# NeymarL/ChineseChess-AlphaZero

Measured on AMD Instinct MI355X. Metric: mcts_node_expansions_per_sec, higher is better.
Workload: dtype f16+2xbf6corr-split/f32acc+f64/i32 tree

## Files before the change

### chinesechess-alphazero_amd/cchess_alphazero/_native.py

```python
import ctypes as C
import os

import numpy as np

_HERE = os.path.dirname(os.path.abspath(__file__))
LIB_PATH = os.environ.get("CZ_LIB") or os.path.join(os.path.dirname(_HERE), "csrc", "libczero.so")

NSQ, NLABELS, MAXMOVES, NOMOVE = 90, 2086, 128, 0xFFFF
F32, F16, BF16, U8, F16C8, F16C6, F16C86 = 0, 1, 2, 3, 4, 5, 6

_lib = None


class NativeError(RuntimeError):
    pass


def lib():
    global _lib
    if _lib is None:
        import torch
        if not os.path.exists(LIB_PATH):
            raise NativeError(
                f"{LIB_PATH} not found: build the HIP engine first "
# ... 34 lines not shown
        L.cz_input_conv.argtypes = [vp, i32, i32, vp, vp, vp, vp, i32, i32, i32, i32, i32, vp]
        L.cz_input_conv.restype = i32
        L.cz_input_conv_packed_elems.argtypes = [i32, i32, i32]
        L.cz_input_conv_packed_elems.restype = C.c_size_t
        L.cz_input_conv_pack_weights.argtypes = [vp, i32, i32, i32, i32, vp]
        L.cz_input_conv_pack_weights.restype = i32
        L.cz_resblock_heads.argtypes = [vp, vp, vp, vp, vp, vp, vp, vp, vp, vp, i32, i32, i32, i32, i32, vp]
        L.cz_resblock_heads.restype = i32
        L.cz_resblock.argtypes = [vp, vp, vp, vp, vp, vp, vp, vp, vp, i32, i32, i32, i32, vp]
        L.cz_input_conv_q.argtypes = [vp, i32, i32, vp, vp, vp, vp, i32, i32, i32, i32, i32, vp, vp, vp]
        L.cz_resblock_q.argtypes = [vp, vp, vp, vp, vp, vp, vp, vp, vp, i32, i32, i32, i32, vp, vp]
        L.cz_resblock_heads_q.argtypes = [vp, vp, vp, vp, vp, vp, vp, vp, vp, vp, i32, i32, i32, i32, i32, vp, vp]
        for _n in ("cz_input_conv_q", "cz_resblock_q", "cz_resblock_heads_q"):
            getattr(L, _n).restype = i32
        L.cz_resblock.restype = i32
        L.cz_split_bias_act.argtypes = [vp, vp, vp, vp, C.c_size_t, i32, i32, i32, i32, vp]
        L.cz_split_bias_act.restype = i32
    if hasattr(L, "cz_conv3x3_c8"):
        L.cz_conv3x3_c8_packed_bytes.argtypes = [i32]
        L.cz_conv3x3_c8_packed_bytes.restype = C.c_size_t
        L.cz_conv3x3_c8_pack_weights.argtypes = [vp, i32, vp]
        L.cz_conv3x3_c8_pack_weights.restype = i32
        L.cz_conv3x3_c6_pack_weights.argtypes = [vp, i32, i32, i32, vp]
        L.cz_conv3x3_c6_pack_weights.restype = i32
        L.cz_conv3x3_c8.argtypes = [vp, vp, vp, vp, vp, vp, vp, vp, vp, i32, i32, i32, vp]
        L.cz_conv3x3_c8.restype = i32
    if hasattr(L, "cz_input_resblock"):
        L.cz_input_resblock.argtypes = [vp, i32, vp, vp, vp, vp, vp, vp, vp, vp, i32, i32, i32, vp, vp, vp]
        L.cz_input_resblock.restype = i32
    if hasattr(L, "cz_tower"):
        L.cz_input_resblock_m.restype = i32
        L.cz_input_resblock_m.argtypes = [vp, vp, i32] + [vp] * 8 + [i32] * 3 + [vp] * 3
        L.cz_tower.restype = i32
        L.cz_tower.argtypes = [vp, vp, i32, vp, vp, vp, vp, vp, vp, i32, vp, vp, vp, vp, vp, vp, i32, i32, i32, vp, vp]
        L.cz_resblock_chain.restype = i32
        L.cz_resblock_chain.argtypes = [vp, vp, i32, vp, vp, vp, vp, vp, vp, vp, i32, i32, i32, vp, vp]
        L.cz_tower_plain.restype = i32
        L.cz_tower_plain.argtypes = [vp, i32, vp, vp, vp, vp, vp, i32, i32, i32, vp, vp]
        L.cz_tower_pairs.restype = i32
        L.cz_tower_pairs.argtypes = [vp, vp, i32, vp, vp, vp, vp, vp, vp, vp, vp, vp, vp, i32, i32, i32, i32, vp, vp]
    if hasattr(L, "cz_heads_tail"):
        L.cz_heads_tail.argtypes = [vp, i32, vp, vp, i32, vp, i32, vp, vp, i32, vp, C.c_float, vp, vp, vp, i32, i32, i32, vp, vp]
        L.cz_heads_tail.restype = i32
        L.cz_fc_packed_elems.argtypes = [i32, i32]
        L.cz_fc_packed_elems.restype = C.c_size_t
        L.cz_fc_pack_weights.argtypes = [vp, i32, i32, i32, vp]
        L.cz_fc_pack_weights.restype = i32
    for name in ("cz_label_tables", "cz_movegen", "cz_done", "cz_step", "cz_encode", "cz_check_or_catch",
                 "cz_be_catched", "cz_has_attack", "cz_rules_fused"):
        getattr(L, name).restype = i32
    if hasattr(L, "cz_replay_games"):
        L.cz_replay_games.argtypes = [vp, vp, vp, i32, i32, vp, vp, vp, vp]
        L.cz_replay_games.restype = i32
    if hasattr(L, "cz_gather_planes"):
        L.cz_gather_planes.argtypes = [vp, vp, i32, vp, i32, i32, vp, vp]
        L.cz_gather_planes.restype = i32
    if hasattr(L, "cz_policy_value_loss"):
        L.cz_policy_value_loss.argtypes = [vp, i32, vp, vp, i32, i32, vp, vp, vp, i32, vp, vp, i32, C.c_float, C.c_float,
                                           vp, vp, vp, vp, vp]
        L.cz_policy_value_loss.restype = i32
    if hasattr(L, "cz_search_create"):
        from . import _native_search
        _native_search.declare(L)


def check(rc, what=""):
# ... 280 lines not shown
    return out_f32 if out_f32 is not None else out


def head_convs(x, w, bias, n_policy, policy_feat, value_feat):
    require_gpu()
    n, c = x.shape[0], x.shape[-1]
    check(lib().cz_head_convs(_ptr(x), _dt_code(x.dtype), _ptr(w), _ptr(bias), _ptr(policy_feat), _ptr(value_feat),
                              n, c, n_policy, w.shape[0] - n_policy, _stream()), "cz_head_convs")
    return policy_feat, value_feat


def input_table(w_oihw):
    import torch
    w = w_oihw.detach().to(torch.float32)
    return w.permute(1, 2, 3, 0).reshape(w.shape[1], 25, w.shape[0]).contiguous()


def input_resblock(planes, table, in_bias, w1, b1, w2, b2, out, rows=None, count=None, masks=None):
    require_gpu()
    import torch
    if planes.dtype != torch.uint8:
        raise NativeError("cz_input_resblock reads uint8 planes")
    n = planes.shape[0]
    if masks is not None:
        assert masks.dtype == torch.int32 and masks.is_cuda and masks.is_contiguous() and tuple(masks.shape) == (n, 96)
    L = lib()
    check(L.cz_input_resblock_m(_ptr(planes), _ptr(masks), planes.shape[1], _ptr(table), _ptr(in_bias), _ptr(w1), _ptr(b1),
                                _ptr(w2), _ptr(b2), _ptr(out[0]), _ptr(out[1]), n, out[0].shape[-1], _pair_code(out),
                                _ptr(rows) if rows is not None else None, _ptr(count) if count is not None else None,
                                _stream()), "cz_input_resblock")
    return out


def pack_fc_weights(w, dtype=None):
    import torch
    dtype = dtype or torch.float16
    w = w.detach().to("cpu", torch.float32).contiguous()
    n = lib().cz_fc_packed_elems(w.shape[0], w.shape[1])
    if n == 0:
        raise NativeError(f"cz_fc_pack_weights: unsupported shape {tuple(w.shape)}")
    out = torch.empty((n,), dtype=dtype)
    check(lib().cz_fc_pack_weights(_ptr(w), w.shape[0], w.shape[1], _dt_code(dtype), _ptr(out)), "cz_fc_pack_weights")
    return out


def heads_tail(policy_feat, value_feat, wp, bias_p, w1, bias1, w2, b2, policy, value, stats, count=None, normalize=True):
    require_gpu()
    n = policy_feat.shape[0]
    check(lib().cz_heads_tail(_ptr(policy_feat), policy_feat.shape[1], _ptr(wp), _ptr(bias_p), policy.shape[1],
                              _ptr(value_feat), value_feat.shape[1], _ptr(w1), _ptr(bias1), bias1.shape[0], _ptr(w2),
                              float(b2), _ptr(policy), _ptr(value), _ptr(stats), n, _dt_code(wp.dtype), int(bool(normalize)),
                              _ptr(count) if count is not None else None, _stream()), "cz_heads_tail")
    return policy, value


def pack_input_conv_weights(w_oihw, dtype, parts):
    import torch
    w = w_oihw.detach().to("cpu", torch.float32).contiguous()
    c, ip = w.shape[0], w.shape[1]
    assert tuple(w.shape[2:]) == (5, 5)
    n = lib().cz_input_conv_packed_elems(c, ip, parts)
    if n == 0:
        raise NativeError(f"cz_input_conv: unsupported channels={c} in_planes={ip} parts={parts}")
    out = torch.empty((n,), dtype=dtype)
    check(lib().cz_input_conv_pack_weights(_ptr(w), c, ip, _dt_code(dtype), parts, _ptr(out)),
          "cz_input_conv_pack_weights")
# ... 150 lines not shown
```

### chinesechess-alphazero_amd/cchess_alphazero/agent/model.py

```python
import hashlib
import json
import os
from logging import getLogger

import torch
import torch.nn as nn
import torch.nn.functional as F

logger = getLogger(__name__)

N_LABELS = 2086
BN_EPS = 1e-3


class ResidualBlock(nn.Module):
    def __init__(self, filters, ksize):
        super().__init__()
        self.conv1 = nn.Conv2d(filters, filters, ksize, padding=ksize // 2, bias=False)
        self.bn1 = nn.BatchNorm2d(filters, eps=BN_EPS, momentum=0.01)
        self.conv2 = nn.Conv2d(filters, filters, ksize, padding=ksize // 2, bias=False)
        self.bn2 = nn.BatchNorm2d(filters, eps=BN_EPS, momentum=0.01)

    def forward(self, x):
        y = F.relu(self.bn1(self.conv1(x)))
# ... 126 lines not shown
        self.c6_blocks = 0
        if arith == "c6" or arith.startswith("c6>"):
            n6 = int(arith[3:]) if arith.startswith("c6>") else nblk
            assert 1 <= n6 <= nblk, arith
            self.c6 = (trunk == "mfma" and dtype == torch.float32 and net.cfg["cnn_filter_num"] in (128, 192) and nblk >= 2)
            if self.c6 and act_exps is None:
                if not from_env:
                    raise ValueError("arith='c6' needs the activation images' exponents: build the network through "
                                     "guarded_inference_net (it measures them on the calibration positions)")
                logger.warning("CZ_TOWER_ARITH=%s without calibrated exponents: using c8 (guarded_inference_net measures them)", arith)
                self.c6 = False
            self.c6_blocks = n6 if self.c6 else 0
            arith = "c8"
        self.act_exps = ([int(v) for v in act_exps[0]], [int(v) for v in act_exps[1]]) if self.c6 else None
        if arith.startswith("c8"):
            c8_blocks = int(arith[3:]) if arith.startswith("c8>") else nblk
            assert 0 <= c8_blocks <= nblk, arith
            if not (trunk == "mfma" and dtype == torch.float32 and net.cfg["cnn_filter_num"] in (128, 192)):
                c8_blocks = 0
            arith = "c8" if c8_blocks else "f16x3"
        assert arith in ("bf16x3", "f16x3", "c8"), arith
        if arith == "f16x3" and not (trunk == "mfma" and dtype == torch.float32):
            arith = "bf16x3"
        self.arith = arith
        self.c8_blocks = c8_blocks
        self.fused_epilogue = True
        self.fused_blocks = True
        self.fused_heads = True
        self.fused_input = os.environ.get("CZ_FUSED_INPUT", "1") != "0"
        self.fused_tail = os.environ.get("CZ_FUSED_TAIL", "1") != "0"
        self.block_events = None
        self.last_plan = None
        self.chain_blocks = os.environ.get("CZ_TOWER_CHAIN", "1") != "0"
        self.chain_heads = os.environ.get("CZ_TOWER_HEADS", "1") != "0"
        self.input_depth = net.cfg["input_depth"]
        self.filters = net.cfg["cnn_filter_num"]
        with torch.no_grad():
            self.input_conv = _fold(net.input_conv, net.input_bn)
            self.res = nn.ModuleList()
            for blk in net.res:
                self.res.append(nn.ModuleList([_fold(blk.conv1, blk.bn1), _fold(blk.conv2, blk.bn2)]))
            self.policy_conv = _fold(net.policy_conv, net.policy_bn)
            self.value_conv = _fold(net.value_conv, net.value_bn)
            self.policy_out = nn.Linear(net.policy_out.in_features, net.policy_out.out_features)
            self.value_dense = nn.Linear(net.value_dense.in_features, net.value_dense.out_features)
            self.value_out = nn.Linear(net.value_out.in_features, 1)
            self.policy_out.load_state_dict(net.policy_out.state_dict())
            self.value_dense.load_state_dict(net.value_dense.state_dict())
            self.value_out.load_state_dict(net.value_out.state_dict())
            self.act_shift = None
            if act_shift is not None and (act_shift[0] != 0 or any(act_shift[1])):
                sx, smid = int(act_shift[0]), [int(v) for v in act_shift[1]]
                assert len(smid) == len(self.res)
                self.act_shift = (sx, smid)
                self.input_conv.weight.mul_(2.0 ** sx)
                self.input_conv.bias.mul_(2.0 ** sx)
                for (c1, c2), sm in zip(self.res, smid):
                    c1.weight.mul_(2.0 ** (sm - sx))
                    c1.bias.mul_(2.0 ** sm)
                    c2.weight.mul_(2.0 ** (sx - sm))
                    c2.bias.mul_(2.0 ** sx)
                self.policy_conv.weight.mul_(2.0 ** -sx)
                self.value_conv.weight.mul_(2.0 ** -sx)
            packed = self._pack_trunk() if trunk == "mfma" else None
        self.to(dtype)
        self.to(memory_format=torch.channels_last)
# ... 172 lines not shown
                cur, tmp, nxt = (self._as_f16_pair(t) for t in (cur, tmp, nxt))
                _native.split_bias_act(last, None, cur, relu=False)
            conv = _native.conv3x3_c8 if i < n8 else _native.conv3x3
            conv(cur, w1, getattr(self, f"tb{i}a"), out=tmp)
            if i + 1 < nblk and i + 1 != n8:
                conv(tmp, w2, getattr(self, f"tb{i}b"), skip=cur, out=nxt)
                cur, nxt = nxt, cur
            elif self.parts == 2:
                conv(tmp, w2, getattr(self, f"tb{i}b"), skip=cur, out_f32=last)
            else:
                conv(tmp, w2, getattr(self, f"tb{i}b"), skip=cur, out=(last,))
        if heads is not None and fused and self.parts == 2 and c == 128:
            return None
        return last

    def block_kinds(self):
        nblk = len(self.res)
        if self.c6:
            return ["c6"] * self.c6_blocks + ["c8"] * (nblk - self.c6_blocks)
        if self.arith == "c8":
            return ["c8"] * self.c8_blocks + ["pair"] * (nblk - self.c8_blocks)
        return ["pair"] * nblk

    def _block_params(self, i):
        od = self.operand_dtype
        return (getattr(self, f"tw{i}a").view(od), getattr(self, f"tb{i}a"), getattr(self, f"tw{i}b").view(od), getattr(self, f"tb{i}b"))

    def _tower_chained(self, planes, cur, nxt, last, heads, rows, count, masks):
        from cchess_alphazero import _native
        kinds = self.block_kinds()
        nblk = len(kinds)
        heads_ok = heads is not None and self.parts == 2 and self.filters == 128
        chain_heads = self.chain_heads and not (kinds[-1] == "pair" and self.operand_dtype == torch.bfloat16)
        key = ("plan", heads_ok, chain_heads, self.tb0a.data_ptr())
        if key not in self._bufs:
            plan = []
            for step in tower_plan(kinds, heads_exit=heads_ok, chain_heads=chain_heads):
                if step[0] in ("tower", "pairs"):
                    blk = step[1]
                    fmt = [_native.IMG_C6 if kinds[blk[0]] == "c6" else _native.IMG_C8] * len(blk)
                    bl = _native.BlockList([self._block_params(i) for i in blk], *((fmt, fmt) if step[0] == "tower" else ()))
                    plan.append(step + (bl,))
                else:
                    plan.append(step)
            self._bufs[key] = plan
        self.last_plan = [st[:3] if st[0] != "first" else st for st in self._bufs[key]]
        img_tag = {"c6": torch.int8, "c8": torch.uint8}

        def view(t, kind):
            if kind == "pair":
                return (t[0], t[1].view(t[0].dtype)) if t[1].dtype in (torch.uint8, torch.int8) else t
            return (t[0], t[1].view(img_tag[kind]))
        fmt_code = {"c6": _native.IMG_C6, "c8": _native.IMG_C8, "pair": _native.IMG_PAIR}
        hd = (self.head_w32, self.head_b32, heads[0], heads[1], heads[2]) if heads_ok else None
        done_heads = False
        for step in self._bufs[key]:
            ev = None
            if self.block_events is not None:
                ev = (torch.cuda.Event(enable_timing=True), torch.cuda.Event(enable_timing=True))
                ev[0].record()
            if step[0] == "first":
                w1, b1, w2, b2 = self._block_params(0)
                _native.input_resblock(planes.contiguous(), self.in_table32, self.in_bias32, w1, b1, w2, b2,
                                       out=view(nxt, kinds[0]), rows=rows, count=count, masks=masks)
                cur, nxt = nxt, cur
                nb = 1
            elif step[0] == "tower":
                _, blk, ex, bl = step
                nb = len(blk)
                if ex == "heads":
                    _native.tower(view(cur, kinds[blk[0]]), bl, _native.EXIT_HEADS, heads=hd, count=count)
                    done_heads = True
                else:
                    _native.tower(view(cur, kinds[blk[0]]), bl, fmt_code[ex], out=view(nxt, ex), count=count)
                    cur, nxt = nxt, cur
            elif step[0] == "pairs":
                _, blk, with_heads, bl = step
                nb = len(blk)
                if with_heads:
                    _native.tower_pairs(view(cur, "pair"), bl, heads=hd, count=count)
                    done_heads = True
                else:
                    _native.tower_pairs(view(cur, "pair"), bl, out=view(nxt, "pair"), count=count)
                    cur, nxt = nxt, cur
            else:
                i = step[1]
                nb = 1
                w1, b1, w2, b2 = self._block_params(i)
                x = view(cur, kinds[i])
                if heads_ok:
                    _native.resblock_heads(x, w1, b1, w2, b2, self.head_w32, self.head_b32, heads[0], heads[1], heads[2],
                                           count=count)
                    done_heads = True
                else:
                    _native.resblock(x, w1, b1, w2, b2, out_f32=last, count=count)
            if ev is not None:
                ev[1].record()
                self.block_events.append(ev + (nb,) if nb > 1 else ev)
        return None if done_heads else last

    def _tower_192(self, cur, nxt, last, count):
        from cchess_alphazero import _native
        kinds = self.block_kinds()
        nblk = len(kinds)
        legacy = os.environ.get("CZ_IP_PAIR", "1")[:1] == "0"
        key = ("plan192", legacy, self.tb0a.data_ptr())
        if key not in self._bufs:
# ... 518 lines not shown
```

### chinesechess-alphazero_amd/csrc/xq_conv.hip

```cpp
#include <hip/hip_runtime.h>
#include <stdint.h>
#include <string.h>
#include <stdlib.h>
#include <stdio.h>
#include <math.h>
#include "../../include/czero.h"
#include "xq_c8_kloop.h"
#include "xq_nn_common.h"

extern "C" void czi_set_error(const char* msg);
extern "C" int czi_pairs4_launch(const void* x_hi, const void* x_lo, int n_blocks, const void* const* w1, const float* const* b1,
                                 const void* const* w2, const float* const* b2, void* y_hi, void* y_lo, const float* head_w,
                                 const float* head_b, float* pol, float* val, int n_pol, int n_boards, int channels, int dtype,
                                 int n_cu, const int32_t* n_dev, void* stream, float* y_f32);

namespace {

struct QueueCtx {
    const int32_t* rows = nullptr;
    const int32_t* n_dev = nullptr;
};
thread_local QueueCtx g_q;

template <int C, int P, int PARTS> struct Geom {
// ... 3285 lines not shown
                               (const unsigned char*)x_img, ch, (_Float16*)y_hi, (unsigned char*)y_img, y_f32, n_boards, n_dev, 0, HeadArgs{});
        else
            hipLaunchKernelGGL((k_resblock_ip4_c8<192, 1, 1>), dim3(blocks), dim3(256), 0, st, (const _Float16*)x_hi,
                               (const unsigned char*)x_img, ch, (_Float16*)y_hi, (unsigned char*)y_img, y_f32, n_boards, n_dev, 0, HeadArgs{});
    } else {
        const unsigned blocks = (unsigned)(n_boards < n_cu ? n_boards : n_cu);
        if (dtype == CZ_F16C8)
            hipLaunchKernelGGL((k_resblock_ip_c8<192, 0, 0>), dim3(blocks), dim3(192 / 32 * 64 + ip::COPY_THREADS), 0, st, (const _Float16*)x_hi,
                               (const unsigned char*)x_img, ch, (_Float16*)y_hi, (unsigned char*)y_img, y_f32, n_boards, n_dev);
        else
            hipLaunchKernelGGL((k_resblock_ip_c8<192, 1, 1>), dim3(blocks), dim3(192 / 32 * 64 + ip::COPY_THREADS), 0, st, (const _Float16*)x_hi,
                               (const unsigned char*)x_img, ch, (_Float16*)y_hi, (unsigned char*)y_img, y_f32, n_boards, n_dev);
    }
    if (hipGetLastError() != hipSuccess) {
        czi_set_error("cz_resblock_chain: launch failed");
        return CZ_ERR_HIP;
    }
    return CZ_OK;
}

extern "C" int czi_tower4_launch(const void* x_hi, const void* x_img, int n_blocks, const void* const* w1, const float* const* b1,
                                 const void* const* w2, const float* const* b2, int c6, int exit_mode, void* y_hi, void* y_img,
                                 const float* head_w, const float* head_b, float* pol, float* val, int n_pol, int n_boards,
                                 int n_cu, const int32_t* n_dev, void* stream)
{
    if (n_blocks > ip::MAX_BLOCKS) return CZ_ERR_ARG;
    const HeadArgs hd{head_w, head_b, pol, val, n_pol};
    hipStream_t st = (hipStream_t)stream;
    ip::Chain ch{};
    ch.n = n_blocks;
    for (int b = 0; b < n_blocks; ++b) { ch.w1[b] = w1[b]; ch.w2[b] = w2[b]; ch.b1[b] = b1[b]; ch.b2[b] = b2[b]; }
    const int n_pairs = (n_boards + 1) / 2;
    const unsigned blocks = (unsigned)(n_pairs < n_cu ? n_pairs : n_cu);
    if (c6)
        hipLaunchKernelGGL((k_resblock_ip4_c8<128, 1, 1>), dim3(blocks), dim3(256), 0, st, (const _Float16*)x_hi, (const unsigned char*)x_img,
                           ch, (_Float16*)y_hi, (unsigned char*)y_img, (float*)nullptr, n_boards, n_dev, exit_mode, hd);
    else
        hipLaunchKernelGGL((k_resblock_ip4_c8<128, 0, 0>), dim3(blocks), dim3(256), 0, st, (const _Float16*)x_hi, (const unsigned char*)x_img,
                           ch, (_Float16*)y_hi, (unsigned char*)y_img, (float*)nullptr, n_boards, n_dev, exit_mode, hd);
    return hipGetLastError() == hipSuccess ? CZ_OK : CZ_ERR_HIP;
}

extern "C" int cz_tower_plain(const void* x, int n_blocks, const void* const* w1_packed, const float* const* bias1,
                              const void* const* w2_packed, const float* const* bias2, void* y, int n_boards, int channels,
                              int dtype, const int32_t* n_dev, void* stream)
{
    if (n_boards < 0 || !x || !y || !w1_packed || !w2_packed || !bias1 || !bias2 || n_blocks < 1 || n_blocks > pl::MAX_BLOCKS ||
        channels != 256 || (dtype != CZ_F16 && dtype != CZ_BF16)) {
        czi_set_error("cz_tower_plain: bad argument (256 filters, plain f16 / bf16 operands, 1 .. 24 blocks)");
        return CZ_ERR_ARG;
    }
    pl::Chain ch{};
    ch.n = n_blocks;
    for (int b = 0; b < n_blocks; ++b) {
        if (!w1_packed[b] || !w2_packed[b] || !bias1[b] || !bias2[b]) {
            czi_set_error("cz_tower_plain: null block parameter");
            return CZ_ERR_ARG;
        }
        ch.w1[b] = w1_packed[b]; ch.w2[b] = w2_packed[b]; ch.b1[b] = bias1[b]; ch.b2[b] = bias2[b];
    }
    if (n_boards == 0) return CZ_OK;
    const int n_cu = device_cu_count();
    if (n_cu < 0) {
        czi_set_error("cz_tower_plain: cannot query the device");
        return CZ_ERR_HIP;
    }
    hipStream_t st = (hipStream_t)stream;
// ... 45 lines not shown
    if (n_cu < 0) {
        czi_set_error("cz_input_resblock: cannot query the device");
        return CZ_ERR_HIP;
    }
    hipStream_t st = (hipStream_t)stream;
    const unsigned blocks = (unsigned)(n_boards < n_cu ? n_boards : n_cu);
    const FirstArgs fa{(const unsigned char*)planes_u8, in_table, in_bias, rows, masks, in_planes, g_first_w1_rounds};
    if (dtype == CZ_F16C6) {
        if (launch_resblock_c8<true, false, true>(nullptr, nullptr, w1_packed, bias1, w2_packed, bias2, y_hi, y_lo, nullptr,
                                                  n_boards, n_cu, st, HeadArgs{}, n_dev, fa) != CZ_OK) {
            czi_set_error("cz_input_resblock: launch failed");
            return CZ_ERR_HIP;
        }
        return CZ_OK;
    }
    if (dtype == CZ_F16C8) {
        if (launch_resblock_c8<true, false>(nullptr, nullptr, w1_packed, bias1, w2_packed, bias2, y_hi, y_lo, nullptr, n_boards,
                                            n_cu, st, HeadArgs{}, n_dev, fa) != CZ_OK) {
            czi_set_error("cz_input_resblock: launch failed");
            return CZ_ERR_HIP;
        }
        return CZ_OK;
    }
    if (dtype == CZ_BF16)
        hipLaunchKernelGGL((k_resblock_pipe<__bf16, true>), dim3(blocks), dim3(512), 0, st, (const __bf16*)nullptr,
                           (const __bf16*)nullptr, (const __bf16*)w1_packed, bias1, (const __bf16*)w2_packed, bias2,
                           (__bf16*)y_hi, (__bf16*)y_lo, n_boards, n_dev, fa);
    else
        hipLaunchKernelGGL((k_resblock_pipe<_Float16, true>), dim3(blocks), dim3(512), 0, st, (const _Float16*)nullptr,
                           (const _Float16*)nullptr, (const _Float16*)w1_packed, bias1, (const _Float16*)w2_packed, bias2,
                           (_Float16*)y_hi, (_Float16*)y_lo, n_boards, n_dev, fa);
    if (hipGetLastError() != hipSuccess) {
        czi_set_error("cz_input_resblock: launch failed");
        return CZ_ERR_HIP;
    }
    return CZ_OK;
}

extern "C" int cz_resblock_pipelined(int enable)
{
    const int old = g_resblock_pipelined;
    if (enable >= 0) g_resblock_pipelined = enable ? 1 : 0;
    return old;
}

extern "C" int cz_input_conv_q(const void* planes, int planes_dtype, int in_planes, const void* w_packed,
                               const float* bias, void* y_hi, void* y_lo, int n_boards, int channels, int dtype,
                               int parts, int relu, const int32_t* rows, const int32_t* n_dev, void* stream)
{
    g_q = QueueCtx{rows, n_dev};
    const int rc = cz_input_conv(planes, planes_dtype, in_planes, w_packed, bias, y_hi, y_lo, n_boards, channels, dtype,
                                 parts, relu, stream);
    g_q = QueueCtx{};
    return rc;
}

extern "C" int cz_resblock_q(const void* x_hi, const void* x_lo, const void* w1_packed, const float* bias1,
                             const void* w2_packed, const float* bias2, void* y_hi, void* y_lo, float* y_f32,
                             int n_boards, int channels, int dtype, int parts, const int32_t* n_dev, void* stream)
{
    g_q = QueueCtx{nullptr, n_dev};
    const int rc = cz_resblock(x_hi, x_lo, w1_packed, bias1, w2_packed, bias2, y_hi, y_lo, y_f32, n_boards, channels,
                               dtype, parts, stream);
    g_q = QueueCtx{};
    return rc;
}
// ... 43 lines not shown
```

### chinesechess-alphazero_amd/csrc/xq_tower.hip

```cpp
#include <hip/hip_runtime.h>
#include <stdint.h>
#include "../../include/czero.h"
#include "xq_c8_kloop.h"
#include "xq_nn_common.h"

extern "C" void czi_set_error(const char* msg);
extern "C" int czi_tower4_launch(const void* x_hi, const void* x_img, int n_blocks, const void* const* w1, const float* const* b1,
                                 const void* const* w2, const float* const* b2, int c6, int exit_mode, void* y_hi, void* y_img,
                                 const float* head_w, const float* head_b, float* pol, float* val, int n_pol, int n_boards,
                                 int n_cu, const int32_t* n_dev, void* stream);

namespace tw4 {
constexpr int MAX_BLOCKS = 12;
struct Chain {
    const void* w1[MAX_BLOCKS];
    const void* w2[MAX_BLOCKS];
    const float* b1[MAX_BLOCKS];
    const float* b2[MAX_BLOCKS];
    int n;
};
}

template <int CH> struct Tp4 {
    static constexpr int C = CH, RB = 2 * CH, CPR = CH / 8, NT = 3, CT = CH / 32, CTW = CT / 2, NTHR = 256, KK = CH / 16;
// ... 323 lines not shown
#undef CZ_P4
    return hipGetLastError() == hipSuccess ? CZ_OK : CZ_ERR_HIP;
}

constexpr int TOWER_MAX_BLOCKS = 8;

static int tower_cu_count()
{
    static int n_cu = 0;
    if (n_cu == 0) {
        int dev = 0;
        hipDeviceProp_t prop;
        if (hipGetDevice(&dev) != hipSuccess || hipGetDeviceProperties(&prop, dev) != hipSuccess) return -1;
        n_cu = prop.multiProcessorCount;
    }
    return n_cu;
}

extern "C" int cz_tower(const void* x_hi, const void* x_img, int n_blocks, const void* const* w1_packed,
                        const float* const* bias1, const void* const* w2_packed, const float* const* bias2,
                        const int* fmt_x, const int* fmt_y, int exit_fmt, void* y_hi, void* y_img, const float* head_w,
                        const float* head_b, float* policy_feat, float* value_feat, int n_policy, int n_value, int n_boards,
                        const int32_t* n_dev, void* stream)
{
    const bool heads = exit_fmt == CZ_EXIT_HEADS;
    if (n_boards < 0 || !x_hi || !x_img || !w1_packed || !w2_packed || !bias1 || !bias2 || n_blocks < 1 ||
        n_blocks > TOWER_MAX_BLOCKS || (!heads && (!y_hi || !y_img)) ||
        (heads && (!head_w || !head_b || !policy_feat || !value_feat || n_policy < 1 || n_value < 1 || n_policy + n_value != 6)) ||
        (!heads && exit_fmt != CZ_IMG_C8 && exit_fmt != CZ_IMG_C6 && exit_fmt != CZ_IMG_PAIR)) {
        czi_set_error("cz_tower: bad argument (1 .. 8 blocks; exit CZ_IMG_C8 / CZ_IMG_C6 / CZ_IMG_PAIR with y_hi + y_img, or "
                      "CZ_EXIT_HEADS with n_policy + n_value == 6)");
        return CZ_ERR_ARG;
    }
    const int fmt0 = fmt_x ? fmt_x[0] : CZ_IMG_C6;
    for (int b = 0; b < n_blocks; ++b) {
        if (!w1_packed[b] || !w2_packed[b] || !bias1[b] || !bias2[b]) {
            czi_set_error("cz_tower: null block parameter");
            return CZ_ERR_ARG;
        }
        const int fx = fmt_x ? fmt_x[b] : CZ_IMG_C6, fy = fmt_y ? fmt_y[b] : CZ_IMG_C6;
        if ((fx != CZ_IMG_C8 && fx != CZ_IMG_C6) || fy != fx || fx != fmt0) {
            czi_set_error("cz_tower: one image format per chain, CZ_IMG_C8 or CZ_IMG_C6 (a hybrid tower is one chain per "
                          "arithmetic -- the exit of the first hands over; pair blocks: cz_tower_pairs)");
            return CZ_ERR_ARG;
        }
    }
    if (!heads && ((fmt0 == CZ_IMG_C6 && exit_fmt == CZ_IMG_PAIR) || (fmt0 == CZ_IMG_C8 && exit_fmt == CZ_IMG_C6))) {
        czi_set_error("cz_tower: a c6 chain ends on a c6 or c8 image, a c8 chain on a c8 image or fp16 pairs");
        return CZ_ERR_ARG;
    }
    if (n_boards == 0) return CZ_OK;
    const int n_cu = tower_cu_count();
    if (n_cu < 0) {
        czi_set_error("cz_tower: cannot query the device");
        return CZ_ERR_HIP;
    }
    const int rc = czi_tower4_launch(x_hi, x_img, n_blocks, w1_packed, bias1, w2_packed, bias2, fmt0 == CZ_IMG_C6,
                                     heads ? 3 : (exit_fmt == CZ_IMG_PAIR ? 2 : 0), y_hi, y_img, head_w, head_b, policy_feat,
                                     value_feat, n_policy, n_boards, n_cu, n_dev, stream);
    if (rc != CZ_OK) czi_set_error("cz_tower: launch failed");
    return rc;
}

extern "C" int cz_tower_pairs(const void* x_hi, const void* x_lo, int n_blocks, const void* const* w1_packed,
                              const float* const* bias1, const void* const* w2_packed, const float* const* bias2, void* y_hi,
                              void* y_lo, const float* head_w, const float* head_b, float* policy_feat, float* value_feat,
                              int n_policy, int n_value, int n_boards, int dtype, const int32_t* n_dev, void* stream)
{
    const bool heads = head_w != nullptr;
    if (n_boards < 0 || !x_hi || !x_lo || !w1_packed || !w2_packed || !bias1 || !bias2 || n_blocks < 1 ||
        n_blocks > TOWER_MAX_BLOCKS || (dtype != CZ_F16 && dtype != CZ_BF16) || (!heads && (!y_hi || !y_lo)) ||
        (heads && (!head_b || !policy_feat || !value_feat || n_policy < 1 || n_value < 1 || n_policy + n_value != 6))) {
        czi_set_error("cz_tower_pairs: bad argument (1 .. 8 blocks of (hi, lo) f16 / bf16 operands; y_hi + y_lo, or the head "
                      "arguments with n_policy + n_value == 6)");
        return CZ_ERR_ARG;
    }
    for (int b = 0; b < n_blocks; ++b) {
        if (!w1_packed[b] || !w2_packed[b] || !bias1[b] || !bias2[b]) {
            czi_set_error("cz_tower_pairs: null block parameter");
            return CZ_ERR_ARG;
        }
    }
    if (n_boards == 0) return CZ_OK;
    const int n_cu = tower_cu_count();
    if (n_cu < 0) {
        czi_set_error("cz_tower_pairs: cannot query the device");
        return CZ_ERR_HIP;
    }
    const int rc = czi_pairs4_launch(x_hi, x_lo, n_blocks, w1_packed, bias1, w2_packed, bias2, y_hi, y_lo, head_w, head_b,
                                     policy_feat, value_feat, n_policy, n_boards, 128, dtype, n_cu, n_dev, stream, nullptr);
// ... 4 lines not shown
```

### include/czero.h

```cpp
#ifndef CZERO_H
#define CZERO_H

#include <stddef.h>
#include <stdint.h>

#ifdef __cplusplus
extern "C" {
#endif

#define CZ_VERSION 2

#define CZ_OK 0
#define CZ_ERR_ARG (-1)
#define CZ_ERR_HIP (-2)
#define CZ_ERR_STATE (-3)
#define CZ_ERR_NOMEM (-4)

#define CZ_NSQ 90
#define CZ_NLABELS 2086
#define CZ_MAXMOVES 128
#define CZ_NOMOVE 0xFFFF

#define CZ_F32 0
#define CZ_F16 1
// ... 102 lines not shown
} cz_visit_entry;
int cz_search_drain_visits(cz_search* s, void* host_buf, int max_entries, int* n_out, uint64_t* dropped_out,
                           void* stream);
int cz_bias_act(void* x, const void* bias, const void* residual, size_t n_elems, int channels, int dtype,
                int relu, void* stream);

int cz_conv3x3(const void* x_hi, const void* x_lo, const void* w_packed, const float* bias, const void* skip_hi,
               const void* skip_lo, void* y_hi, void* y_lo, float* y_f32, int n_boards, int channels, int dtype,
               int parts, int relu, void* stream);
int cz_resblock(const void* x_hi, const void* x_lo, const void* w1_packed, const float* bias1, const void* w2_packed,
                const float* bias2, void* y_hi, void* y_lo, float* y_f32, int n_boards, int channels, int dtype,
                int parts, void* stream);
size_t cz_conv3x3_c8_packed_bytes(int channels);
int cz_conv3x3_c8_pack_weights(const float* w_oihw, int channels, void* out_host);
int cz_conv3x3_c8(const void* x_hi, const void* x_c8, const void* w_packed, const float* bias,
                  const void* skip_hi, const void* skip_c8, void* y_hi, void* y_c8, float* y_f32,
                  int n_boards, int channels, int relu, void* stream);

int cz_conv3x3_c6_pack_weights(const float* w_oihw, int channels, int x_exp, int y_exp, void* out_host);

int cz_resblock_pipelined(int enable);
int cz_resblock_heads(const void* x_hi, const void* x_lo, const void* w1_packed, const float* bias1,
                      const void* w2_packed, const float* bias2, const float* head_w, const float* head_b,
                      float* policy_feat, float* value_feat, int n_boards, int channels, int dtype, int n_policy,
                      int n_value, void* stream);
int cz_input_resblock(const void* planes_u8, int in_planes, const float* in_table, const float* in_bias,
                      const void* w1_packed, const float* bias1, const void* w2_packed, const float* bias2, void* y_hi,
                      void* y_lo, int n_boards, int channels, int dtype, const int32_t* rows, const int32_t* n_dev,
                      void* stream);
int cz_input_resblock_m(const void* planes_u8, const uint32_t* masks, int in_planes, const float* in_table,
                        const float* in_bias, const void* w1_packed, const float* bias1, const void* w2_packed,
                        const float* bias2, void* y_hi, void* y_lo, int n_boards, int channels, int dtype,
                        const int32_t* rows, const int32_t* n_dev, void* stream);
size_t cz_conv3x3_packed_elems(int channels, int parts);
int cz_conv3x3_pack_weights(const float* w_oihw, int channels, int dtype, int parts, void* out_host);
int cz_input_conv(const void* planes, int planes_dtype, int in_planes, const void* w_packed, const float* bias,
                  void* y_hi, void* y_lo, int n_boards, int channels, int dtype, int parts, int relu, void* stream);
size_t cz_input_conv_packed_elems(int channels, int in_planes, int parts);
int cz_input_conv_q(const void* planes, int planes_dtype, int in_planes, const void* w_packed, const float* bias,
                    void* y_hi, void* y_lo, int n_boards, int channels, int dtype, int parts, int relu,
                    const int32_t* rows, const int32_t* n_dev, void* stream);
int cz_resblock_q(const void* x_hi, const void* x_lo, const void* w1_packed, const float* bias1, const void* w2_packed,
                  const float* bias2, void* y_hi, void* y_lo, float* y_f32, int n_boards, int channels, int dtype,
                  int parts, const int32_t* n_dev, void* stream);
#define CZ_IMG_C8 0
#define CZ_IMG_C6 1
#define CZ_IMG_PAIR 2
#define CZ_EXIT_HEADS 3
int cz_tower(const void* x_hi, const void* x_img, int n_blocks, const void* const* w1_packed, const float* const* bias1,
             const void* const* w2_packed, const float* const* bias2, const int* fmt_x, const int* fmt_y, int exit_fmt,
             void* y_hi, void* y_img, const float* head_w, const float* head_b, float* policy_feat, float* value_feat,
             int n_policy, int n_value, int n_boards, const int32_t* n_dev, void* stream);
int cz_tower_pairs(const void* x_hi, const void* x_lo, int n_blocks, const void* const* w1_packed, const float* const* bias1,
                   const void* const* w2_packed, const float* const* bias2, void* y_hi, void* y_lo, const float* head_w,
                   const float* head_b, float* policy_feat, float* value_feat, int n_policy, int n_value, int n_boards,
                   int dtype, const int32_t* n_dev, void* stream);
int cz_resblock_chain(const void* x_hi, const void* x_img, int n_blocks, const void* const* w1_packed, const float* const* bias1,
                      const void* const* w2_packed, const float* const* bias2, void* y_hi, void* y_img, float* y_f32, int n_boards,
                      int channels, int dtype, const int32_t* n_dev, void* stream);
int cz_tower_plain(const void* x, int n_blocks, const void* const* w1_packed, const float* const* bias1,
                   const void* const* w2_packed, const float* const* bias2, void* y, int n_boards, int channels, int dtype,
                   const int32_t* n_dev, void* stream);
int cz_resblock_heads_q(const void* x_hi, const void* x_lo, const void* w1_packed, const float* bias1,
                        const void* w2_packed, const float* bias2, const float* head_w, const float* head_b,
                        float* policy_feat, float* value_feat, int n_boards, int channels, int dtype, int n_policy,
                        int n_value, const int32_t* n_dev, void* stream);
// ... 34 lines not shown
```

Baseline: 1.820 million.

## Split input conv into standalone gather kernel and fold block 0 into tower chain

Adds a dedicated input-gather kernel that computes only the sparse input convolution (table lookups per occupied plane/tap) and writes a c8 image. The first residual block then runs inside the persistent tower kernel, which gains a mode where block 0 reads a c8 image while the rest of the chain stays c6. The aim is to replace the fused input+resblock kernel with a lighter gather plus a longer chained tower, giving the first block the tower's more efficient code path. In exchange it adds an extra intermediate image round trip and a new kernel variant.

```diff
diff --git a/chinesechess-alphazero_amd/cchess_alphazero/_native.py b/chinesechess-alphazero_amd/cchess_alphazero/_native.py
--- a/chinesechess-alphazero_amd/cchess_alphazero/_native.py
+++ b/chinesechess-alphazero_amd/cchess_alphazero/_native.py
@@ -90,6 +90,8 @@
         L.cz_input_resblock_m.restype = i32
         L.cz_input_resblock_m.argtypes = [vp, vp, i32] + [vp] * 8 + [i32] * 3 + [vp] * 3
         L.cz_tower.restype = i32
+        L.cz_input_gather.restype = i32
+        L.cz_input_gather.argtypes = [vp, vp, i32, vp, vp, vp, vp, i32, vp, vp, vp]
         L.cz_tower.argtypes = [vp, vp, i32, vp, vp, vp, vp, vp, vp, i32, vp, vp, vp, vp, vp, vp, i32, i32, i32, vp, vp]
         L.cz_resblock_chain.restype = i32
         L.cz_resblock_chain.argtypes = [vp, vp, i32, vp, vp, vp, vp, vp, vp, vp, i32, i32, i32, vp, vp]
@@ -436,6 +438,21 @@
     return out
 
 
+def input_gather(planes, table, in_bias, out, rows=None, count=None, masks=None):
+    require_gpu()
+    import torch
+    if planes.dtype != torch.uint8:
+        raise NativeError("cz_input_gather reads uint8 planes")
+    n = planes.shape[0]
+    if masks is not None:
+        assert masks.dtype == torch.int32 and masks.is_cuda and masks.is_contiguous() and tuple(masks.shape) == (n, 96)
+    assert out[0].dtype == torch.float16 and out[1].dtype in (torch.uint8, torch.int8) and out[0].shape[-1] == 128
+    check(lib().cz_input_gather(_ptr(planes), _ptr(masks), planes.shape[1], _ptr(table), _ptr(in_bias), _ptr(out[0]),
+                                _ptr(out[1]), n, _ptr(rows) if rows is not None else None,
+                                _ptr(count) if count is not None else None, _stream()), "cz_input_gather")
+    return out
+
+
 def pack_fc_weights(w, dtype=None):
     import torch
     dtype = dtype or torch.float16
diff --git a/chinesechess-alphazero_amd/cchess_alphazero/agent/model.py b/chinesechess-alphazero_amd/cchess_alphazero/agent/model.py
--- a/chinesechess-alphazero_amd/cchess_alphazero/agent/model.py
+++ b/chinesechess-alphazero_amd/cchess_alphazero/agent/model.py
@@ -182,6 +182,8 @@
         self.block_events = None
         self.last_plan = None
         self.chain_blocks = os.environ.get("CZ_TOWER_CHAIN", "1") != "0"
+        self.first_in_chain = os.environ.get("CZ_TOWER_FIRST", "1") != "0"
+        self.last_launches = None
         self.chain_heads = os.environ.get("CZ_TOWER_HEADS", "1") != "0"
         self.input_depth = net.cfg["input_depth"]
         self.filters = net.cfg["cnn_filter_num"]
@@ -420,19 +422,28 @@
         nblk = len(kinds)
         heads_ok = heads is not None and self.parts == 2 and self.filters == 128
         chain_heads = self.chain_heads and not (kinds[-1] == "pair" and self.operand_dtype == torch.bfloat16)
-        key = ("plan", heads_ok, chain_heads, self.tb0a.data_ptr())
+        steps = tower_plan(kinds, heads_exit=heads_ok, chain_heads=chain_heads)
+        gather = (self.first_in_chain and kinds[0] == "c6" and planes.shape[1] <= 14 and steps[1][0] == "tower" and
+                  kinds[steps[1][1][0]] == "c6" and len(steps[1][1]) < 8)
+        key = ("plan", heads_ok, chain_heads, gather, self.tb0a.data_ptr())
         if key not in self._bufs:
-            plan = []
-            for step in tower_plan(kinds, heads_exit=heads_ok, chain_heads=chain_heads):
+            plan, launches = [], []
+            for step in steps:
                 if step[0] in ("tower", "pairs"):
                     blk = step[1]
                     fmt = [_native.IMG_C6 if kinds[blk[0]] == "c6" else _native.IMG_C8] * len(blk)
-                    bl = _native.BlockList([self._block_params(i) for i in blk], *((fmt, fmt) if step[0] == "tower" else ()))
+                    run, fx = blk, fmt
+                    if gather and step is steps[1]:
+                        run, fx = [0] + blk, [_native.IMG_C8] + fmt
+                    bl = _native.BlockList([self._block_params(i) for i in run], *((fx, [fmt[0]] * len(run)) if step[0] == "tower" else ()))
                     plan.append(step + (bl,))
+                    launches.append((step[0], run, step[2]))
                 else:
                     plan.append(step)
-            self._bufs[key] = plan
-        self.last_plan = [st[:3] if st[0] != "first" else st for st in self._bufs[key]]
+                    launches.append(("gather", [], "c8") if step[0] == "first" and gather else (step[0], [step[1]], None))
+            self._bufs[key] = plan, launches
+        plan, self.last_launches = self._bufs[key]
+        self.last_plan = [st[:3] if st[0] != "first" else st for st in plan]
         img_tag = {"c6": torch.int8, "c8": torch.uint8}
 
         def view(t, kind):
@@ -442,12 +453,17 @@
         fmt_code = {"c6": _native.IMG_C6, "c8": _native.IMG_C8, "pair": _native.IMG_PAIR}
         hd = (self.head_w32, self.head_b32, heads[0], heads[1], heads[2]) if heads_ok else None
         done_heads = False
-        for step in self._bufs[key]:
+        for step in plan:
             ev = None
             if self.block_events is not None:
                 ev = (torch.cuda.Event(enable_timing=True), torch.cuda.Event(enable_timing=True))
                 ev[0].record()
-            if step[0] == "first":
+            if step[0] == "first" and gather:
+                _native.input_gather(planes.contiguous(), self.in_table32, self.in_bias32, out=view(nxt, "c8"), rows=rows,
+                                     count=count, masks=masks)
+                cur, nxt = nxt, cur
+                nb = 1
+            elif step[0] == "first":
                 w1, b1, w2, b2 = self._block_params(0)
                 _native.input_resblock(planes.contiguous(), self.in_table32, self.in_bias32, w1, b1, w2, b2,
                                        out=view(nxt, kinds[0]), rows=rows, count=count, masks=masks)
@@ -456,11 +472,12 @@
             elif step[0] == "tower":
                 _, blk, ex, bl = step
                 nb = len(blk)
+                x = view(cur, "c8" if bl.n > nb else kinds[blk[0]])
                 if ex == "heads":
-                    _native.tower(view(cur, kinds[blk[0]]), bl, _native.EXIT_HEADS, heads=hd, count=count)
+                    _native.tower(x, bl, _native.EXIT_HEADS, heads=hd, count=count)
                     done_heads = True
                 else:
-                    _native.tower(view(cur, kinds[blk[0]]), bl, fmt_code[ex], out=view(nxt, ex), count=count)
+                    _native.tower(x, bl, fmt_code[ex], out=view(nxt, ex), count=count)
                     cur, nxt = nxt, cur
             elif step[0] == "pairs":
                 _, blk, with_heads, bl = step
diff --git a/chinesechess-alphazero_amd/csrc/xq_conv.hip b/chinesechess-alphazero_amd/csrc/xq_conv.hip
--- a/chinesechess-alphazero_amd/csrc/xq_conv.hip
+++ b/chinesechess-alphazero_amd/csrc/xq_conv.hip
@@ -3341,7 +3341,11 @@
     for (int b = 0; b < n_blocks; ++b) { ch.w1[b] = w1[b]; ch.w2[b] = w2[b]; ch.b1[b] = b1[b]; ch.b2[b] = b2[b]; }
     const int n_pairs = (n_boards + 1) / 2;
     const unsigned blocks = (unsigned)(n_pairs < n_cu ? n_pairs : n_cu);
-    if (c6)
+    if (c6 == 2)
+        hipLaunchKernelGGL((k_resblock_ip4_c8<128, 1, 1, true>), dim3(blocks), dim3(256), 0, st, (const _Float16*)x_hi,
+                           (const unsigned char*)x_img, ch, (_Float16*)y_hi, (unsigned char*)y_img, (float*)nullptr, n_boards, n_dev,
+                           exit_mode, hd);
+    else if (c6)
         hipLaunchKernelGGL((k_resblock_ip4_c8<128, 1, 1>), dim3(blocks), dim3(256), 0, st, (const _Float16*)x_hi, (const unsigned char*)x_img,
                            ch, (_Float16*)y_hi, (unsigned char*)y_img, (float*)nullptr, n_boards, n_dev, exit_mode, hd);
     else
@@ -3453,6 +3457,155 @@
                            (_Float16*)y_hi, (_Float16*)y_lo, n_boards, n_dev, fa);
     if (hipGetLastError() != hipSuccess) {
         czi_set_error("cz_input_resblock: launch failed");
+        return CZ_ERR_HIP;
+    }
+    return CZ_OK;
+}
+
+namespace ig {
+constexpr int C = 128, HALF = 64, MAX_PLANES = 14, WAVES = 16, NTHR = WAVES * 64, NP = 2;
+constexpr int MASK_OFF = MAX_PLANES * 25 * HALF * 4, LDS_BYTES = MASK_OFF + WAVES * 96 * 4;
+static_assert(LDS_BYTES <= 160 * 1024, "a table half + the waves' occupancy boards must fit the CU's LDS");
+}
+
+__global__ __launch_bounds__(ig::NTHR, 1) void k_input_gather_c8(FirstArgs fa, _Float16* __restrict__ yh,
+                                                                  unsigned char* __restrict__ yc, int n_boards,
+                                                                  const int32_t* __restrict__ n_dev)
+{
+    using namespace ig;
+    __shared__ __attribute__((aligned(16))) unsigned char lds[ig::LDS_BYTES];
+    if (n_dev) {
+        const int nd = __builtin_amdgcn_readfirstlane(*n_dev);
+        n_boards = nd < n_boards ? nd : n_boards;
+    }
+    const int tid = threadIdx.x, lane = tid & 63, wave = tid >> 6;
+    const int half = blockIdx.x & 1, groups = gridDim.x >> 1, grp = blockIdx.x >> 1;
+    float4* tab = reinterpret_cast<float4*>(lds);
+    for (int i = tid; i < fa.in_planes * 25 * 16; i += NTHR)
+        tab[i] = reinterpret_cast<const float4*>(fa.table + (size_t)(i >> 4) * C + half * HALF)[i & 15];
+    __syncthreads();
+    uint32_t* mk = reinterpret_cast<uint32_t*>(lds + MASK_OFF) + wave * 96;
+    const uint32_t plane_bits = fa.in_planes < 32 ? (1u << fa.in_planes) - 1u : ~0u;
+    const int sub = lane & 15, ps = lane >> 4;
+    const int ch0 = half * HALF + sub * 4;
+    const float4 bias = *reinterpret_cast<const float4*>(fa.in_bias + ch0);
+    for (int b = grp * WAVES + wave; b < n_boards; b += groups * WAVES) {
+        const size_t slot = (size_t)(fa.rows ? fa.rows[b] : b);
+        if (fa.masks) {
+            mk[lane] = fa.masks[slot * 96 + lane] & plane_bits;
+            if (lane < 32) mk[64 + lane] = fa.masks[slot * 96 + 64 + lane] & plane_bits;
+        } else {
+            mk[lane] = 0u;
+            if (lane < 32) mk[64 + lane] = 0u;
+            asm volatile("s_waitcnt lgkmcnt(0)" ::: "memory");
+            __builtin_amdgcn_wave_barrier();
+            const int words = fa.in_planes * 90 / 4;
+            const uint32_t* src = reinterpret_cast<const uint32_t*>(fa.planes + slot * (size_t)(fa.in_planes * 90));
+            for (int w = lane; w < words; w += 64) {
+                const uint32_t word = src[w];
+                if (word == 0u) continue;
+                int c = (w * 4) / 90, pix = w * 4 - c * 90;
+#pragma unroll
+                for (int k4 = 0; k4 < 4; ++k4) {
+                    if ((word >> (8 * k4)) & 0xFFu) atomicOr(&mk[pix], 1u << c);
+                    if (++pix == 90) { pix = 0; ++c; }
+                }
+            }
+        }
+        asm volatile("s_waitcnt lgkmcnt(0)" ::: "memory");
+        __builtin_amdgcn_wave_barrier();
+        const uint64_t occ_lo = __ballot(mk[lane] != 0u);
+        const uint64_t occ_hi = __ballot(lane < 26 && mk[64 + (lane & 31)] != 0u);
+        for (int j = 0; j < 90; j += 4 * NP) {
+            float acc[NP][4];
+            uint32_t occ[NP], cur_m[NP];
+            int cur_tap[NP];
+#pragma unroll
+            for (int s = 0; s < NP; ++s) {
+                acc[s][0] = bias.x; acc[s][1] = bias.y; acc[s][2] = bias.z; acc[s][3] = bias.w;
+                const int p = j + 4 * s + ps;
+                const int py = p / 9, px = p - py * 9;
+                uint32_t o = 0u;
+                if (p < 90) {
+#pragma unroll
+                    for (int ky = 0; ky < 5; ++ky) {
+                        const int r = py + ky - 2;
+                        if ((unsigned)r < 10u) {
+                            const int sh = r * 9;
+                            const uint32_t rowbits = (uint32_t)((sh < 64 ? (occ_lo >> sh) | (sh > 55 ? occ_hi << (64 - sh) : 0ull)
+                                                                         : occ_hi >> (sh - 64)) & 0x1FFull);
+                            o |= (((rowbits << 2) >> px) & 31u) << (5 * ky);
+                        }
+                    }
+                }
+                occ[s] = o;
+                cur_m[s] = 0u;
+                cur_tap[s] = 0;
+            }
+            for (;;) {
+                uint32_t any = 0u;
+#pragma unroll
+                for (int s = 0; s < NP; ++s) {
+                    if (cur_m[s] == 0u && occ[s] != 0u) {
+                        const int tap = __builtin_ctz(occ[s]);
+                        occ[s] &= occ[s] - 1u;
+                        cur_tap[s] = tap;
+                        cur_m[s] = mk[j + 4 * s + ps + (tap / 5 - 2) * 9 + (tap % 5 - 2)];
+                    }
+                    any |= cur_m[s];
+                }
+                if (!__ballot(any != 0u)) break;
+                float4 w[NP];
+#pragma unroll
+                for (int s = 0; s < NP; ++s)
+                    if (cur_m[s]) w[s] = tab[(__builtin_ctz(cur_m[s]) * 25 + cur_tap[s]) * 16 + sub];
+#pragma unroll
+                for (int s = 0; s < NP; ++s)
+                    if (cur_m[s]) {
+                        acc[s][0] += w[s].x; acc[s][1] += w[s].y; acc[s][2] += w[s].z; acc[s][3] += w[s].w;
+                        cur_m[s] &= cur_m[s] - 1u;
+                    }
+            }
+#pragma unroll
+            for (int s = 0; s < NP; ++s) {
+                const int p = j + 4 * s + ps;
+                if (p >= 90) continue;
+                float r[4];
+#pragma unroll
+                for (int i = 0; i < 4; ++i) r[i] = acc[s][i] > 0.0f ? acc[s][i] : 0.0f;
+                const cf8::Split4 o = cf8::split4(r);
+                const size_t q = (size_t)b * 90 + p;
+                *reinterpret_cast<Quad<_Float16>*>(yh + q * C + ch0) = o.hi;
+                *reinterpret_cast<uint32_t*>(yc + q * 2 * C + ch0) = o.l8;
+                *reinterpret_cast<uint32_t*>(yc + q * 2 * C + C + ch0) = o.h8;
+            }
+        }
+        __builtin_amdgcn_wave_barrier();
+    }
+}
+
+extern "C" int cz_input_gather(const void* planes_u8, const uint32_t* masks, int in_planes, const float* in_table,
+                               const float* in_bias, void* y_hi, void* y_img, int n_boards, const int32_t* rows,
+                               const int32_t* n_dev, void* stream)
+{
+    if (n_boards < 0 || (!planes_u8 && !masks) || !in_table || !in_bias || !y_hi || !y_img || in_planes < 1 ||
+        in_planes > ig::MAX_PLANES || (in_planes * 90) % 4 != 0) {
+        czi_set_error("cz_input_gather: bad argument (u8 planes or occupancy boards, in_planes even and <= 14)");
+        return CZ_ERR_ARG;
+    }
+    if (n_boards == 0) return CZ_OK;
+    const int n_cu = device_cu_count();
+    if (n_cu < 0) {
+        czi_set_error("cz_input_gather: cannot query the device");
+        return CZ_ERR_HIP;
+    }
+    const int want = (n_boards + ig::WAVES - 1) / ig::WAVES, cap = n_cu / 2 > 0 ? n_cu / 2 : 1;
+    const unsigned blocks = 2u * (unsigned)(want < cap ? want : cap);
+    const FirstArgs fa{(const unsigned char*)planes_u8, in_table, in_bias, rows, masks, in_planes, 0};
+    hipLaunchKernelGGL(k_input_gather_c8, dim3(blocks), dim3(ig::NTHR), 0, (hipStream_t)stream, fa, (_Float16*)y_hi,
+                       (unsigned char*)y_img, n_boards, n_dev);
+    if (hipGetLastError() != hipSuccess) {
+        czi_set_error("cz_input_gather: launch failed");
         return CZ_ERR_HIP;
     }
     return CZ_OK;
diff --git a/chinesechess-alphazero_amd/csrc/xq_tower.hip b/chinesechess-alphazero_amd/csrc/xq_tower.hip
--- a/chinesechess-alphazero_amd/csrc/xq_tower.hip
+++ b/chinesechess-alphazero_amd/csrc/xq_tower.hip
@@ -379,16 +379,18 @@
                       "CZ_EXIT_HEADS with n_policy + n_value == 6)");
         return CZ_ERR_ARG;
     }
-    const int fmt0 = fmt_x ? fmt_x[0] : CZ_IMG_C6;
+    const bool mix = fmt_x && fmt_y && fmt_x[0] == CZ_IMG_C8 && fmt_y[0] == CZ_IMG_C6;
+    const int fmt0 = mix ? CZ_IMG_C6 : (fmt_x ? fmt_x[0] : CZ_IMG_C6);
     for (int b = 0; b < n_blocks; ++b) {
         if (!w1_packed[b] || !w2_packed[b] || !bias1[b] || !bias2[b]) {
             czi_set_error("cz_tower: null block parameter");
             return CZ_ERR_ARG;
         }
-        const int fx = fmt_x ? fmt_x[b] : CZ_IMG_C6, fy = fmt_y ? fmt_y[b] : CZ_IMG_C6;
+        const int fx = mix && b == 0 ? CZ_IMG_C6 : (fmt_x ? fmt_x[b] : CZ_IMG_C6), fy = fmt_y ? fmt_y[b] : CZ_IMG_C6;
         if ((fx != CZ_IMG_C8 && fx != CZ_IMG_C6) || fy != fx || fx != fmt0) {
             czi_set_error("cz_tower: one image format per chain, CZ_IMG_C8 or CZ_IMG_C6 (a hybrid tower is one chain per "
-                          "arithmetic -- the exit of the first hands over; pair blocks: cz_tower_pairs)");
+                          "arithmetic -- the exit of the first hands over; pair blocks: cz_tower_pairs; a c6 chain's block 0 "
+                          "may read a c8 image)");
             return CZ_ERR_ARG;
         }
     }
@@ -402,7 +404,7 @@
         czi_set_error("cz_tower: cannot query the device");
         return CZ_ERR_HIP;
     }
-    const int rc = czi_tower4_launch(x_hi, x_img, n_blocks, w1_packed, bias1, w2_packed, bias2, fmt0 == CZ_IMG_C6,
+    const int rc = czi_tower4_launch(x_hi, x_img, n_blocks, w1_packed, bias1, w2_packed, bias2, mix ? 2 : fmt0 == CZ_IMG_C6,
                                      heads ? 3 : (exit_fmt == CZ_IMG_PAIR ? 2 : 0), y_hi, y_img, head_w, head_b, policy_feat,
                                      value_feat, n_policy, n_boards, n_cu, n_dev, stream);
     if (rc != CZ_OK) czi_set_error("cz_tower: launch failed");
diff --git a/include/czero.h b/include/czero.h
--- a/include/czero.h
+++ b/include/czero.h
@@ -158,6 +158,8 @@
                         const float* in_bias, const void* w1_packed, const float* bias1, const void* w2_packed,
                         const float* bias2, void* y_hi, void* y_lo, int n_boards, int channels, int dtype,
                         const int32_t* rows, const int32_t* n_dev, void* stream);
+int cz_input_gather(const void* planes_u8, const uint32_t* masks, int in_planes, const float* in_table, const float* in_bias,
+                    void* y_hi, void* y_img, int n_boards, const int32_t* rows, const int32_t* n_dev, void* stream);
 size_t cz_conv3x3_packed_elems(int channels, int parts);
 int cz_conv3x3_pack_weights(const float* w_oihw, int channels, int dtype, int parts, void* out_host);
 int cz_input_conv(const void* planes, int planes_dtype, int in_planes, const void* w_packed, const float* bias,
```

New measurement: 1.766 million (median of 2 runs). -3.0%, worse.
